# Bergvca/string_grouper

Hardware: NVIDIA H100
Metric: match_strings matched pairs/sec (663k names self-match @0.8, top 20, 3-gram) (higher is better)
Workload: dtype f64

## Files before the change

include/sg_b200.h:

```cpp
#ifndef SG_B200_H
#define SG_B200_H

#include <stddef.h>
#include <stdint.h>

#ifdef __cplusplus
extern "C" {
#endif

#define SG_OK 0
#define SG_ERR_INVALID (-1)
#define SG_ERR_CUDA (-2)
#define SG_ERR_OVERFLOW (-3)
#define SG_ERR_UNSUPPORTED (-4)

#define SG_DTYPE_F32 0
#define SG_DTYPE_F64 1

#define SG_FLAG_IGNORE_CASE 1u
#define SG_FLAG_STRIP_DEFAULT 2u

const char *sg_last_error(void);
int sg_abi_version(void);
int sg_device_info(int *sm_count, int *smem_optin_bytes, int *l2_bytes);

int64_t sg_tfidf_table_slots(int ngram);
int sg_tfidf_count(const uint8_t *bytes , const int64_t *offsets ,
                   int64_t n_docs, int ngram, unsigned flags, int32_t *df_table ,
                   uint8_t *scratch_clean , uint32_t *scratch_sort ,
                   uint32_t *scratch_key , uint32_t *scratch_tf ,
                   int32_t *row_nnz , void *stream);

size_t sg_tfidf_vocab_workspace_bytes(int64_t n_docs, int ngram);
int sg_tfidf_vocab(int64_t n_docs, int ngram, const int32_t *df_table , int32_t *rank_table ,
                   int32_t *row_nnz , int64_t *indptr ,
                   int32_t *vocab_size , int64_t *nnz_total , void *ws ,
                   size_t ws_bytes, void *stream);
int sg_tfidf_values(const int64_t *offsets , int64_t n_docs, int dtype,
                    const void *idf , const int32_t *rank_table ,
                    const uint32_t *scratch_key, const uint32_t *scratch_tf, const int32_t *row_nnz,
                    const int64_t *indptr , int32_t *indices ,
                    double *val64 , float *val32 , void *stream);

int sg_tfidf_vocab_keys(const int32_t *df_table , const int32_t *rank_table , int ngram,
                        uint32_t *keys_out , void *stream);
int sg_tfidf_vocab_df(const int32_t *df_table , const int32_t *rank_table , int ngram,
                      int32_t *df_out , void *stream);

int sg_tfidf64_count(const void *symbols , int sym_width, const int64_t *offsets ,
                     int64_t n_docs, int ngram, int bits, const uint8_t *lut ,
                     uint32_t *scratch_clean , uint64_t *scratch_sort ,
                     uint64_t *scratch_key , uint32_t *scratch_tf ,
                     int32_t *row_nnz , void *stream);
size_t sg_tfidf64_vocab_workspace_bytes(int64_t n_docs, int64_t total_symbols);
int sg_tfidf64_vocab(const int64_t *offsets , int64_t n_docs, int64_t total_symbols, int ngram, int bits,
                     const uint64_t *scratch_key, int32_t *row_nnz, int64_t *indptr ,
                     int32_t *indices , uint64_t *vocab_keys ,
                     int32_t *df , int32_t *vocab_size , int64_t *nnz_total ,
                     void *ws , size_t ws_bytes, void *stream);
int sg_tfidf64_values(const int64_t *offsets , int64_t n_docs, int dtype,
                      const void *idf , const uint32_t *scratch_tf,
                      const int64_t *indptr , const int32_t *indices ,
                      double *val64 , float *val32 , void *stream);

#define SG_SYMBOL_UNKNOWN 0xffffffffu
#define SG_LUT_UNKNOWN 0xfeu
int sg_tfidf_transform_count(const uint8_t *bytes , const int64_t *offsets ,
                             int64_t n_docs, int ngram, unsigned flags, uint8_t *scratch_clean ,
                             uint32_t *scratch_sort , uint32_t *scratch_key ,
                             uint32_t *scratch_tf , int32_t *row_nnz , void *stream);
size_t sg_tfidf_transform_workspace_bytes(int64_t n_docs);
int sg_tfidf_known(const int64_t *offsets , int64_t n_docs, const int32_t *df_table ,
                   uint32_t *scratch_key , uint32_t *scratch_tf , int32_t *row_nnz ,
                   int64_t *indptr , void *ws , size_t ws_bytes, void *stream);
int sg_tfidf64_transform_count(const void *symbols , int sym_width, const int64_t *offsets ,
                               int64_t n_docs, int ngram, int bits, const uint8_t *lut ,
                               uint32_t *scratch_clean, uint64_t *scratch_sort, uint64_t *scratch_key,
                               uint32_t *scratch_tf, int32_t *row_nnz , void *stream);
int sg_tfidf64_known(const int64_t *offsets , int64_t n_docs, const uint64_t *vocab_keys ,
                     int32_t vocab_size, const uint64_t *scratch_key , uint32_t *scratch_tf ,
// ... 325 lines not shown
```

string_grouper_b200/_device.py:

```python
import ctypes
import math
import os

import numpy as np

from . import _lib

_TORCH = None

LAUNCH_COUNTS = {"postings": 0, "candidates": 0, "rescore": 0, "select": 0, "symmetrize": 0, "tfidf": 0,
                 "rowdot": 0, "order": 0, "tiles": 0, "groups": 0, "gather": 0, "prune": 0, "dedup": 0,
                 "nearest": 0, "fields": 0}

TRANSFER_BYTES = {"d2h": 0, "h2d": 0}

DEFAULT_TILE_W = int(os.environ.get("SG_B200_TILE_W", "0"))
DEFAULT_WARPS = int(os.environ.get("SG_B200_WARPS", "8"))
GROUP_BYTES = int(os.environ.get("SG_B200_GROUP_MB", "6")) << 20
CAND_MARGIN = 1.5e-3
U16_MARGIN_PER_FEATURE = 2e-5
PRUNE_FRAC = float(os.environ.get("SG_B200_PRUNE", "0.9"))
ACC_DTYPE = os.environ.get("SG_B200_ACC", "u16")
MAX_CAND_DENSITY = float(os.environ.get("SG_B200_MAX_CAND_DENSITY", "1.5e-3"))
MAX_BUCKETS = int(os.environ.get("SG_B200_MAX_BUCKETS", str(400_000_000)))
# ... 304 lines not shown


def _build_postings(B, perm, tile_w, n_spilled=None):
    t = require_cuda()
    L = _lib.load()
    n_rows, n_cols = B.shape
    T = int(L.sg_num_tiles(n_rows, tile_w))
    nb = T * (n_cols + 1)
    if nb >= 2**31 - 1:
        raise OverflowError("posting bucket table too large: %d features x %d tiles" % (n_cols, T))
    Tp = int(L.sg_num_tiles_padded(n_rows, tile_w))
    bucket_dir = _empty(2 * nb, t.int32, B.device)
    bucket_maxw = _empty((n_cols + 1) * Tp, t.float16, B.device)
    post = _empty(max(B.nnz, 1), t.int32, B.device)
    ws_bytes = int(L.sg_postings_workspace_bytes(B.nnz, n_cols, T))
    ws = _empty(ws_bytes, t.uint8, B.device)
    w_scale = candidate_scales(1.0, B.norm_bound)[0]
    _lib.check(L.sg_postings_build(n_rows, n_cols, B.nnz, _ptr(B.d_indptr), _ptr(B.d_indices), _ptr(B.d_val32),
                                   _ptr(perm), tile_w, B.base, w_scale,
                                   _ptr(bucket_dir), _ptr(bucket_maxw), _ptr(post), _ptr(n_spilled),
                                   _ptr(ws), ws_bytes, _stream()))
    LAUNCH_COUNTS["postings"] += 5
    bound = t.zeros(Tp, dtype=t.float32, device=B.device)
    _lib.check(L.sg_tile_bounds(n_rows, _ptr(perm), _ptr(B._heavy_norm), tile_w, _ptr(bound), _stream()))
    LAUNCH_COUNTS["prune"] += 1
    return bucket_dir, bucket_maxw, post, T, bound


class DeviceMatches:

    def __init__(self, shape, row, col, score, nnz, max_row, out_dtype=np.float64, indptr=None):
        self.shape = (int(shape[0]), int(shape[1]))
        self.d_row, self.d_col, self.d_score, self.d_indptr = row, col, score, indptr
        self.nnz = int(nnz)
        self.max_row = int(max_row)
        self.out_dtype = np.dtype(out_dtype)
        self._host = None
        self.pending_fix_diagonal = False
        self.pending_mirror = False

    def with_pending(self, fix_diagonal=False, mirror=False):
        self.pending_fix_diagonal |= bool(fix_diagonal)
        self.pending_mirror |= bool(mirror)
        return self

    def host_triples(self):
        n = self.nnz
        t = torch()
        return tuple(to_host(self.d_row[:n].to(t.int64), self.d_col[:n].to(t.int64), self.d_score[:n]))

    def to_scipy(self):
        if self._host is None:
            from scipy.sparse import csr_matrix
            r, c, s = self.host_triples()
            indptr = np.zeros(self.shape[0] + 1, dtype=np.int64)
            np.cumsum(np.bincount(r, minlength=self.shape[0]), out=indptr[1:])
            idx_dtype = np.int32 if max(self.shape) < 2**31 and self.nnz < 2**31 else np.int64
            self._host = csr_matrix((s.astype(self.out_dtype, copy=False), c.astype(idx_dtype),
                                     indptr.astype(idx_dtype)), shape=self.shape)
        return self._host

    def get_shape(self):
        return self.shape

    def toarray(self):
        return self.to_scipy().toarray()

    def __getattr__(self, name):
        if name in _SCIPY_CSR_ATTRS:
            return getattr(self.to_scipy(), name)
        raise AttributeError("%s has no attribute %r" % (type(self).__name__, name))

# ... 238 lines not shown
        stats["dedup"] = groups is not None

    mark(stats, "k2_start")
    scale = A.norm_bound * B.norm_bound
    margin = CAND_MARGIN * max(scale, 1.0)
    thr_c = max(float(threshold) - margin, 0.0)
    acc = (acc or ACC_DTYPE).lower()
    if acc not in ("u16", "f32"):
        raise ValueError("accumulator dtype must be 'u16' or 'f32', got %r" % (acc,))
    if not fixed_point_ok(A, B) or thr_c < 0.05:
        acc = "f32"
    acc_code = _lib.SG_ACC_U16 if acc == "u16" else _lib.SG_ACC_F32
    margin_pf = U16_MARGIN_PER_FEATURE if acc == "u16" else 0.0
    kernel = (kernel or K2_KERNEL).lower()
    if kernel not in ("tiles", "row"):
        raise ValueError("kernel must be 'tiles' or 'row', got %r" % (kernel,))
    use_tiles = kernel == "tiles" and acc == "u16" and B.shape[1] <= int(L.sg_tiles_max_cols())
    tiles = None
    if use_tiles:
        tiles = right_tiles(B)
        if tiles["stage_bytes"] is None:
            tiles["stage_bytes"] = int(tiles["maxima"][0].item())
        smem_optin = t.cuda.get_device_properties(dev).shared_memory_per_block_optin
        tile_warps = next((w for w in (TILE_WARPS, 8) if w in (8, 16) and
                           int(L.sg_tiles_smem_bytes(tiles["stage_bytes"], w)) <= smem_optin), None)
        if tile_warps is None:
            use_tiles, tiles = False, None
    if use_tiles:
        margin = TILE_MARGIN * max(scale, 1.0)
        margin_pf = TILE_MARGIN_PER_FEATURE
    _, a_scale, b_scale = candidate_scales(A.norm_bound, B.norm_bound)
    prune_auto = prune is None
    prune = PRUNE_FRAC if prune is None else float(prune)
    counters = t.zeros(4, dtype=t.int64, device=dev)
    cap = int(os.environ.get("SG_B200_CAND_CAP", 0)) or min(96 * n_rows + (1 << 22), 1 << 30)
    if use_tiles:
        hrank, perm_b, _ = right_order(B)
        tile_w, warps, T, tile_bound = tiles["W"], tile_warps, tiles["T"], tiles["bound"]
        tiles_per_group = 0
        lpack = _empty(2 * A.d_indices.numel(), t.int32, dev)
        mask_words = int(L.sg_tiles_mask_words(n_right))
    else:
        tile_w, warps = pick_tile(n_right, tile_w, warps, 2 if acc == "u16" else 4, n_left=n_rows)
        if blocked:
            warps = 8
        while (-(-n_right // tile_w)) * (B.shape[1] + 1) > MAX_BUCKETS and tile_w < 32768:
            tile_w *= 2
        if blocked:
            hrank, perm_b, rank_b, bucket_dir, bucket_maxw, post, T, tile_bound, sorted_ids = \
                blocked_right_side(B, ids_b, tile_w)
        else:
            hrank, perm_b, _, bucket_dir, bucket_maxw, post, T, tile_bound = right_side(B, tile_w)
        tiles_per_group = max(64, int(GROUP_BYTES // max(4 * B.nnz / T, 1)) // 64 * 64)
    triangle = not nearest and A is B and row_begin == 0 and row_end == n_left
    hi_pos = None
    if blocked:
        lo_pos, hi_pos = block_ranges(sorted_ids, ids_a)
        if triangle:
            perm_a, diag_rank = perm_b, rank_b
        else:
            perm_a = blocked_order(row_order(A, hrank, row_begin, row_end, want_rank=False)[0], ids_a)
            diag_rank = lo_pos
        pair_cum = np.zeros(n_rows + 1, dtype=np.int64)
        pair_cum[1:] = to_host(t.cumsum((hi_pos - diag_rank)[perm_a.long()].long(), 0))[0]
    elif triangle:
        perm_a, diag_rank = perm_b, right_order(B)[2]
    else:
        perm_a, _ = row_order(A, hrank, row_begin, row_end, want_rank=False)
        diag_rank = None
    mark(stats, "right_side")
    c_count = ctypes.c_void_p(counters.data_ptr())
    c_queue = ctypes.c_void_p(counters.data_ptr() + 8)
    c_walk = ctypes.c_void_p(counters.data_ptr() + 16)
    c_mirror = ctypes.c_void_p(counters.data_ptr() + 24) if triangle else None
    dummy = _empty(1, t.int32, dev)
    pruned = {}
    group_items = None
    if blocked:
        group_items = _empty(2 * -(-T // tiles_per_group) + 1, t.int64, dev)
    elif triangle and not use_tiles:
        group_items = _empty(-(-T // tiles_per_group) + 1, t.int64, dev)

    def launch_tiles(perm, n, row_buf, col_buf, capacity):
        l_idx, l_val, l_len, l_thr, l_xp, _ = pruned["arrays"]
        stride = (n + 31) // 32 * 32
        rowinfo = _empty(4 * stride, t.int32, dev)
        mask = _empty(mask_words * stride, t.int32, dev)
        diag_tile_min = _empty(stride // 32, t.int32, dev) if triangle else None
        counters.zero_()
        _lib.check(L.sg_tiles_pack_left(n, _ptr(perm), 0, _ptr(A.d_indptr), _ptr(l_len), _ptr(l_idx), _ptr(l_val),
                                        _ptr(l_thr), _ptr(l_xp), max(B.norm_bound, 1.0), _ptr(lpack), _ptr(rowinfo),
                                        _stream()))
        _lib.check(L.sg_tiles_filter(n, _ptr(rowinfo), _ptr(lpack), _ptr(tiles["maxw"]), n_right, _ptr(tile_bound),
                                     _ptr(perm), _ptr(diag_rank), _ptr(diag_tile_min), _ptr(mask), stride, _stream()))
        _lib.check(L.sg_tiles_candidates(_ptr(perm), n, 0, _ptr(rowinfo), _ptr(lpack), _ptr(mask), stride,
                                         _ptr(tiles["desc"]), _ptr(tiles["blob"]), n_right, B.shape[1],
                                         _ptr(tile_bound), _ptr(perm_b), _ptr(diag_rank), _ptr(diag_tile_min),
                                         tiles["stage_bytes"], _ptr(row_buf), _ptr(col_buf), capacity, c_count,
                                         c_queue, c_walk, warps, _stream()))
        LAUNCH_COUNTS["tiles"] += 3

    def launch(perm, rb, re_, row_buf, col_buf, capacity, partial_buf=None):
        if use_tiles:
            return launch_tiles(perm, re_ - rb, row_buf, col_buf, capacity)
        l_idx, l_val, l_len, l_thr, l_xp, _ = pruned["arrays"]
        counters.zero_()
        if blocked:
            _lib.check(L.sg_cossim_candidates_range(
                _ptr(A.d_indptr), _ptr(l_len), _ptr(l_idx), _ptr(l_val), rb, re_, _ptr(perm), n_right, A.shape[1],
                _ptr(bucket_dir), _ptr(bucket_maxw), _ptr(post), _ptr(perm_b), tile_w, acc_code,
                a_scale, b_scale, thr_c, _ptr(l_thr), _ptr(l_xp), _ptr(tile_bound), tiles_per_group,
                _ptr(diag_rank), _ptr(hi_pos), _ptr(group_items), _ptr(row_buf), _ptr(col_buf), _ptr(partial_buf),
                capacity, c_count, c_queue, warps, _stream()))
            LAUNCH_COUNTS["candidates"] += 1
            return
        _lib.check(L.sg_cossim_candidates(
            _ptr(A.d_indptr), _ptr(l_len), _ptr(l_idx), _ptr(l_val), rb, re_, _ptr(perm), n_right,
            A.shape[1], _ptr(bucket_dir), _ptr(bucket_maxw), _ptr(post), _ptr(perm_b), tile_w, acc_code,
            a_scale, b_scale, thr_c, _ptr(l_thr), _ptr(l_xp), _ptr(tile_bound), tiles_per_group, _ptr(diag_rank),
            _ptr(group_items), _ptr(row_buf), _ptr(col_buf), _ptr(partial_buf), capacity, c_count, c_queue, warps,
            _stream()))
        LAUNCH_COUNTS["candidates"] += 1

    levels = [prune]
    if prune_auto and prune > 0.0 and thr_c > 0.0:
        levels = [prune, 0.75 * prune, 0.5 * prune, 0.25 * prune, 0.0]

    def prepare(level):
        if (level > 0.0 and thr_c > 0.0) or margin_pf > 0.0:
            pruned["arrays"] = prune_left(A, B, hrank, row_begin, row_end, float(threshold), margin, margin_pf,
                                          level if thr_c > 0.0 else 0.0)
        else:
            pruned["arrays"] = (A.d_indices, A.d_val32, None, None, None, None)

    def timed_launch(perm, rb, re_, row_buf, col_buf, capacity, partial_buf=None):
        if _timed(stats):
            ev0, ev1 = t.cuda.Event(enable_timing=True), t.cuda.Event(enable_timing=True)
            ev0.record()
        launch(perm, rb, re_, row_buf, col_buf, capacity, partial_buf)
        if _timed(stats):
            ev1.record()
            stats.setdefault("candidate_events", []).append((ev0, ev1))
        head = counters[:4].cpu().numpy()
        if use_tiles and stats is not None:
            stats["pairs_walked"] = stats.get("pairs_walked", 0) + int(head[2])
            stats["postings_walked"] = stats.get("postings_walked", 0) + int(head[3])
        return int(head[0])

    fixed_cap = bool(os.environ.get("SG_B200_CAND_CAP"))
    sample = None
    if not fixed_cap and n_rows >= 65536:
        stride = max(64, n_rows // 8192)
        sample = perm_a[:n_rows:stride].contiguous()
    est = None
    first = None
    search = True
    n_pairs = (float(pair_cum[-1]) if blocked else n_rows * (n_rows + 1) / 2 if triangle
               else float(n_rows) * n_right)
    dense = MAX_CAND_DENSITY * n_pairs

    def share(lo, hi):
        if blocked:
            return float(pair_cum[hi] - pair_cum[lo]) / max(n_pairs, 1.0)
        if not triangle:
            return (hi - lo) / n_rows
        return ((hi - lo) * n_rows - (lo + hi - 1) * (hi - lo) / 2) / (n_rows * (n_rows + 1) / 2)

    chunk_cand = max(CAND_CHUNK // 2, 1) if triangle else CAND_CHUNK
    refine = REFINE and not use_tiles and acc == "u16" and margin_pf > 0.0
    if not fixed_cap and (n_pairs if blocked else float(n_rows) * float(n_right)) <= OPTIMISTIC_PAIRS:
        prune = levels[0]
        prepare(prune)
        cap0 = int(min(int(dense) + (1 << 22), chunk_cand))
        cand_row0 = _empty(cap0, t.int32, dev)
        cand_col0 = _empty(cap0, t.int32, dev)
        cand_part0 = _empty(cap0, t.float32, dev) if refine else None
        mark(stats, "prune_sample")
        n0 = timed_launch(perm_a, row_begin, row_end, cand_row0, cand_col0, cap0, cand_part0)
        mark(stats, "candidates")
        too_dense = len(levels) > 1 and sample is not None and n0 > dense
        if n0 <= cap0 and not too_dense:
            first = (cand_row0, cand_col0, cand_part0, n0)
            search = False
        else:
            del cand_row0, cand_col0, cand_part0
            if _timed(stats):
                stats["wasted_launch"] = True
            if too_dense:
                levels = levels[1:]
            else:
                est, search = n0, False
    if search:
        for level in levels:
            prepare(level)
            prune = level
            if sample is None:
                break
            launch(sample, row_begin, row_begin + int(sample.numel()), dummy, dummy, 0)
            est = int(counters[0].item()) * stride
            if est <= dense:
                break
    l_idx, l_val, l_len, l_thr, l_xp, l_xg = pruned["arrays"]
    mark(stats, "prune_sample")
    if stats is not None:
        stats["prune"], stats["acc"] = prune, acc
        stats["kernel"] = "tiles" if use_tiles else "row"
        stats["n_candidates_estimate"] = est
        kept_len = (l_len[row_begin:row_end] if l_len is not None else
                    A.d_indptr[row_begin + 1:row_end + 1] - A.d_indptr[row_begin:row_end])
        stats["n_rows_long"] = int((kept_len > 32).sum().item())
        if stats.get("count_macs") and l_len is not None:
            df = feature_df(B).long()
            pos = t.arange(A.d_indices.numel(), device=dev)
            rid = t.searchsorted(A.d_indptr[:n_left + 1].contiguous(), pos, right=True) - 1
            ok = (rid >= row_begin) & (rid < row_end)
            rid = rid.clamp(0, n_left - 1)
            live = ok & ((pos - A.d_indptr[rid]) < l_len[rid].long())
            stats["macs_walked"] = int(df[l_idx.long().clamp(0, A.shape[1] - 1)][live].sum().item())
            stats["features_kept"] = int(live.sum().item())

    n_chunks = 1 if est is None else max(1, -(-int(1.3 * est) // chunk_cand))
    rows_per_chunk = -(-n_rows // n_chunks)
    kept = []
    n_cand_total = n_above = 0
    max_row_cnt = 0
    row_cnt = t.zeros(n_rows + 1, dtype=t.int32, device=dev)
    for lo in range(0, n_rows, rows_per_chunk):
        hi = min(lo + rows_per_chunk, n_rows)
        perm_chunk = perm_a if (lo == 0 and hi == n_rows) else perm_a[lo:hi]
        if est is not None:
            cap = min(max(int(1.3 * est * share(lo, hi)) + (1 << 22), 1 << 22), 1 << 31)
        for attempt in range(3):
            if first is not None:
                cand_row, cand_col, cand_part, n_cand = first
                first = None
                break
            cand_row = _empty(cap, t.int32, dev)
            cand_col = _empty(cap, t.int32, dev)
            cand_part = _empty(cap, t.float32, dev) if refine else None
            n_cand = timed_launch(perm_chunk, row_begin, row_begin + (hi - lo), cand_row, cand_col, cap, cand_part)
            if n_cand <= cap:
                break
            if n_cand * 24 > t.cuda.get_device_properties(dev).total_memory // 2:
                raise OverflowError("%d candidate pairs above the threshold do not fit the candidate buffer; "
                                    "raise min_similarity or split the input" % n_cand)
            cap = n_cand
        else:
            raise OverflowError("candidate buffer overflow")
        n_cand_total += n_cand
        mark(stats, "candidates")
        n_out = 2 * n_cand if triangle else n_cand
        score = _empty(n_out, t.float64, dev)
        keep_row = _empty(n_out, t.int32, dev)
        keep_col = _empty(n_out, t.int32, dev)
        counters.zero_()
        if nearest and refine and cand_part is not None and l_xg is not None:
            _lib.check(L.sg_rescore_refined_nearest(
                n_cand, _ptr(cand_row), _ptr(cand_col), _ptr(cand_part), _ptr(l_xg), _ptr(B._heavy_groups),
                _ptr(l_thr), _ptr(A.d_indptr), _ptr(A.d_indices), _ptr(A.d_val), _ptr(B.d_indptr), _ptr(B.d_indices),
                _ptr(B.d_val), dt, _ptr(score), float(threshold), _ptr(keep_row), _ptr(keep_col), c_count, c_walk,
                _ptr(row_best), row_begin, None, None, 0.0, 0.0, None, _stream()))
        elif nearest:
            _lib.check(L.sg_rescore_nearest(n_cand, _ptr(cand_row), _ptr(cand_col), _ptr(A.d_indptr),
                                            _ptr(A.d_indices), _ptr(A.d_val), _ptr(B.d_indptr), _ptr(B.d_indices),
                                            _ptr(B.d_val), dt, _ptr(score), float(threshold), _ptr(keep_row),
                                            _ptr(keep_col), c_count, _ptr(row_best), row_begin, None, None, _stream()))
        elif refine and cand_part is not None and l_xg is not None:
            _lib.check(L.sg_rescore_refined(n_cand, _ptr(cand_row), _ptr(cand_col), _ptr(cand_part), _ptr(l_xg),
                                            _ptr(B._heavy_groups), _ptr(l_thr), _ptr(A.d_indptr), _ptr(A.d_indices),
                                            _ptr(A.d_val), _ptr(B.d_indptr), _ptr(B.d_indices), _ptr(B.d_val), dt,
                                            _ptr(score), float(threshold), _ptr(keep_row), _ptr(keep_col), c_count,
                                            c_walk, c_mirror, _ptr(row_cnt), row_begin, _stream()))
        else:
            _lib.check(L.sg_rescore(n_cand, _ptr(cand_row), _ptr(cand_col), _ptr(A.d_indptr), _ptr(A.d_indices),
                                    _ptr(A.d_val), _ptr(B.d_indptr), _ptr(B.d_indices), _ptr(B.d_val), dt,
                                    _ptr(score), float(threshold), _ptr(keep_row), _ptr(keep_col), c_count,
                                    c_mirror, _ptr(row_cnt), row_begin, _stream()))
        LAUNCH_COUNTS["rescore"] += 1
        if lo + rows_per_chunk >= n_rows:
            _lib.check(L.sg_row_count_max(n_rows, _ptr(row_cnt), c_queue, _stream()))
        head = counters[:4].cpu().numpy()
        n_keep, max_row_cnt = int(head[0]), int(head[1])
        n_above += n_keep - int(head[3])
        if refine and stats is not None:
            stats["n_refined"] = stats.get("n_refined", 0) + int(head[2])
        mark(stats, "rescore")
        if n_chunks > 1:
            keep_row, keep_col, score = keep_row[:n_keep].clone(), keep_col[:n_keep].clone(), score[:n_keep].clone()
# ... 424 lines not shown
        LAUNCH_COUNTS["select"] += 7
        if stats is not None:
            stats["select"] = "sort"
    th = tail.cpu().numpy()
    mark(stats, "select")
    nnz = int(th[0])
    max_row = int(th[1:2].view(np.int32)[0])
    return DeviceMatches(shape, out_row, out_col, out_score, nnz, max_row, indptr=out_indptr)


def _select_groups(cand_row, cand_col, score, n_cand, groups, top_n, shape, stats):
    t = torch()
    L = _lib.load()
    dev = cand_row.device
    m, n = groups["m"], shape[0]
    grp_cnt = _empty(m, t.int32, dev)
    totals = t.zeros(2, dtype=t.int64, device=dev)
    _lib.check(L.sg_topn_groups_count(n_cand, _ptr(cand_row), _ptr(cand_col), m, _ptr(groups["mem_ptr"]), top_n,
                                      _ptr(grp_cnt), _ptr(totals), _stream()))
    n_expanded, n_out = (int(x) for x in totals.cpu().numpy())
    out_indptr = _empty(n + 1, t.int64, dev)
    out_row = _empty(n_out, t.int32, dev)
    out_col = _empty(n_out, t.int32, dev)
    out_score = _empty(n_out, t.float64, dev)
    tail = t.zeros(2, dtype=t.int64, device=dev)
    ws_bytes = int(L.sg_topn_select_groups_workspace_bytes(n_cand, n_expanded, m, n, top_n))
    ws = _empty(ws_bytes, t.uint8, dev)
    _lib.check(L.sg_topn_select_groups(n_cand, _ptr(cand_row), _ptr(cand_col), _ptr(score), m, _ptr(groups["mem_ptr"]),
                                       _ptr(groups["mem_rows"]), _ptr(grp_cnt), n_expanded, n, _ptr(groups["uid"]),
                                       top_n, _ptr(out_indptr), _ptr(out_row), _ptr(out_col), _ptr(out_score),
                                       ctypes.c_void_p(tail.data_ptr()), ctypes.c_void_p(tail.data_ptr() + 8),
                                       _ptr(ws), ws_bytes, _stream()))
    LAUNCH_COUNTS["select"] += 11 if top_n <= 32 else 13
    th = tail.cpu().numpy()
    mark(stats, "select")
    if stats is not None:
        stats["select"] = "rows"
        stats["n_unique_rows"], stats["n_expanded"] = m, n_expanded
    nnz = int(th[0])
    max_row = int(th[1:2].view(np.int32)[0])
    return DeviceMatches(shape, out_row, out_col, out_score, nnz, max_row, indptr=out_indptr)


def symmetrize(M, fix_diagonal=True, mirror=True):
    t = require_cuda()
    L = _lib.load()
    n = M.shape[0]
    dev = M.d_row.device
    flags = (_lib.SG_SYMM_FIX_DIAGONAL if fix_diagonal else 0) | (_lib.SG_SYMM_MIRROR if mirror else 0)
    cap = 2 * M.nnz + n
    out_row = _empty(cap, t.int32, dev)
    out_col = _empty(cap, t.int32, dev)
    out_score = _empty(cap, t.float64, dev)
    out_nnz = t.zeros(1, dtype=t.int64, device=dev)
    ws_bytes = int(L.sg_symmetrize_workspace_bytes(M.nnz, n))
    ws = _empty(ws_bytes, t.uint8, dev)
    _lib.check(L.sg_symmetrize(n, M.nnz, flags, _ptr(M.d_row), _ptr(M.d_col), _ptr(M.d_score), _ptr(out_row),
                               _ptr(out_col), _ptr(out_score), _ptr(out_nnz), _ptr(ws), ws_bytes, _stream()))
    LAUNCH_COUNTS["symmetrize"] += 3
    nnz = int(out_nnz.item())
    return DeviceMatches(M.shape, out_row, out_col, out_score, nnz, M.max_row, out_dtype=M.out_dtype)


def group_reps(M, n, centroid, keep_device=False):
    t = require_cuda()
    L = _lib.load()
    dev = M.d_row.device
    rep = _empty(n, t.int32, dev)
    ws_bytes = int(L.sg_group_reps_workspace_bytes(n))
    ws = _empty(ws_bytes, t.uint8, dev)
    _lib.check(L.sg_group_reps(n, M.nnz, _ptr(M.d_row), _ptr(M.d_col), _ptr(M.d_score), 1 if centroid else 0,
                               _ptr(rep), _ptr(ws), ws_bytes, _stream()))
    LAUNCH_COUNTS["groups"] += 6
    host = rep[:n].cpu().numpy().astype(np.int64)
    return (host, rep) if keep_device else host


def group_star(M, n, centroid, keep_device=False):
    t = require_cuda()
    L = _lib.load()
    dev = M.d_row.device
    rep = _empty(n, t.int32, dev)
    ws_bytes = int(L.sg_group_star_workspace_bytes(n))
    ws = _empty(ws_bytes, t.uint8, dev)
    _lib.check(L.sg_group_star(n, M.nnz, _ptr(M.d_row), _ptr(M.d_col), _ptr(M.d_score), 1 if centroid else 0,
                               _ptr(rep), _ptr(ws), ws_bytes, _stream()))
    LAUNCH_COUNTS["groups"] += 7 if centroid else 3
    host = rep[:n].cpu().numpy().astype(np.int64)
    return (host, rep) if keep_device else host


def nearest_master(M, n_right):
    t = require_cuda()
    L = _lib.load()
# ... 102 lines not shown
        k, n_rows, ptrs(*[p.d_indptr.data_ptr() for p in parts]), ptrs(*[p.d_indices.data_ptr() for p in parts]),
        ptrs(*[p.d_val.data_ptr() for p in parts]), (ctypes.c_double * k)(*[float(s) for s in scales]),
        (ctypes.c_int32 * k)(*[int(c) for c in col_off[:-1]]), _lib.SG_DTYPE_F64 if f64 else _lib.SG_DTYPE_F32,
        _ptr(indptr), _ptr(indices), _ptr(val), _ptr(val32) if f64 else None, _ptr(ws), ws_bytes, _stream()))
    LAUNCH_COUNTS["fields"] += 2
    return DeviceCSR((n_rows, int(col_off[-1])), indptr, indices, val, val32, nnz, np_dtype, 1.0)


def pair_scores(A, B, M):
    t = require_cuda()
    L = _lib.load()
    if not M.nnz:
        return np.zeros(0, np.float64)
    out = _empty(M.nnz, t.float64, M.d_row.device)
    dt = _lib.SG_DTYPE_F32 if A.dtype == np.float32 else _lib.SG_DTYPE_F64
    _lib.check(L.sg_rescore(M.nnz, _ptr(M.d_row), _ptr(M.d_col), _ptr(A.d_indptr), _ptr(A.d_indices), _ptr(A.d_val),
                            _ptr(B.d_indptr), _ptr(B.d_indices), _ptr(B.d_val), dt, _ptr(out), 0.0, None, None, None,
                            None, None, 0, _stream()))
    LAUNCH_COUNTS["rescore"] += 1
    return to_host(out[:M.nnz])[0]


def sklearn_idf(df, n_docs_fit, dtype):
    dtype = np.float32 if np.dtype(dtype) == np.float32 else np.float64
    df = np.asarray(df).astype(dtype)
    df += 1.0
    idf = np.full_like(df, fill_value=int(n_docs_fit) + 1, dtype=dtype)
    idf /= df
    np.log(idf, out=idf)
    idf += 1.0
    return idf


def _upload_idf(df_host, n_docs_fit, np_dtype, device):
    idf = sklearn_idf(df_host, n_docs_fit, np_dtype)
    TRANSFER_BYTES["h2d"] += int(idf.nbytes)
    d_idf = torch().from_numpy(idf).to(device) if len(idf) else _empty(1, torch().float64, device)
    return idf, d_idf


class DeviceVocabulary:

    alphabet = np.arange(128, dtype=np.uint32)
    bits = 7

    def __init__(self, df_table, rank_table, ngram, n_docs, vocab_size, idf=None, d_idf=None):
        self.d_df, self.d_rank = df_table, rank_table
        self.ngram, self.n_docs, self.size = int(ngram), int(n_docs), int(vocab_size)
        self.idf_, self.d_idf = idf, d_idf
        self._sorted_keys = None

    def sorted_keys(self):
        if self._sorted_keys is None:
            t = require_cuda()
            L = _lib.load()
            keys = _empty(self.size, t.int32, self.d_df.device)
            _lib.check(L.sg_tfidf_vocab_keys(_ptr(self.d_df), _ptr(self.d_rank), self.ngram, _ptr(keys), _stream()))
            self._sorted_keys = keys.to(t.int64)
            LAUNCH_COUNTS["tfidf"] += 1
        return self._sorted_keys

    def feature_names(self):
        from ._ingest import decode_vocab_keys
        t = require_cuda()
        L = _lib.load()
        keys = _empty(self.size, t.int32, self.d_df.device)
        _lib.check(L.sg_tfidf_vocab_keys(_ptr(self.d_df), _ptr(self.d_rank), self.ngram, _ptr(keys), _stream()))
        return decode_vocab_keys(keys[:self.size].cpu().numpy().view(np.uint32), self.ngram)


def upload_strings(data, offsets, device=None):
    t = require_cuda()
    device = device or t.device("cuda", t.cuda.current_device())
    total = int(offsets[-1])
    d_bytes = (t.from_numpy(np.ascontiguousarray(data)).to(device, non_blocking=True) if total
               else _empty(1, t.uint8, device))
    d_off = t.from_numpy(np.ascontiguousarray(offsets, dtype=np.int64)).to(device, non_blocking=True)
    return d_bytes, d_off, total


class DeviceVocabulary64:

    def __init__(self, keys, df, alphabet, bits, ngram, n_docs, vocab_size, idf=None, d_idf=None):
# ... 111 lines not shown
    slots = int(L.sg_tfidf_table_slots(int(ngram)))
    if slots < 0:
        raise NotImplementedError("ngram_size=%r: the device vectoriser supports 1 <= ngram_size <= 4" % (ngram,))
    np_dtype = np.float32 if np.dtype(dtype) == np.float32 else np.float64
    df = t.zeros(slots, dtype=t.int32, device=device)
    rank = _empty(slots, t.int32, device)
    s_clean = _empty(total, t.uint8, device)
    s_sort = _empty(total, t.int32, device)
    s_key = _empty(total, t.int32, device)
    s_tf = _empty(total, t.int32, device)
    row_nnz = _empty(n_docs + 1, t.int32, device)
    _lib.check(L.sg_tfidf_count(_ptr(d_bytes), _ptr(d_off), n_docs, int(ngram), int(flags), _ptr(df), _ptr(s_clean),
                                _ptr(s_sort), _ptr(s_key), _ptr(s_tf), _ptr(row_nnz), _stream()))
    if df_allreduce is not None:
        df_allreduce(df)
    indptr = _empty(n_docs + 1, t.int64, device)
    indices = _empty(total, t.int32, device)
    val32 = _empty(total, t.float32, device)
    val64 = _empty(total, t.float64, device) if np_dtype == np.float64 else None
    tail = t.zeros(2, dtype=t.int64, device=device)
    ws_bytes = int(L.sg_tfidf_vocab_workspace_bytes(n_docs, int(ngram)))
    ws = _empty(ws_bytes, t.uint8, device)
    dt = _lib.SG_DTYPE_F32 if np_dtype == np.float32 else _lib.SG_DTYPE_F64
    _lib.check(L.sg_tfidf_vocab(n_docs, int(ngram), _ptr(df), _ptr(rank), _ptr(row_nnz), _ptr(indptr),
                                ctypes.c_void_p(tail.data_ptr()), ctypes.c_void_p(tail.data_ptr() + 8), _ptr(ws),
                                ws_bytes, _stream()))
    n_master = int(n_master)
    head = t.cat([tail, indptr[n_master:n_master + 1]]).cpu().numpy()
    V = int(head[0:1].view(np.int32)[0])
    nnz = int(head[1])
    split = int(head[2])
    n_fit = n_docs if n_docs_fit is None else int(n_docs_fit)
    col_df = _empty(max(V, 1), t.int32, device)
    _lib.check(L.sg_tfidf_vocab_df(_ptr(df), _ptr(rank), int(ngram), _ptr(col_df), _stream()))
    idf, d_idf = _upload_idf(to_host(col_df[:V])[0], n_fit, np_dtype, device)
    _lib.check(L.sg_tfidf_values(_ptr(d_off), n_docs, dt, _ptr(d_idf), _ptr(rank), _ptr(s_key), _ptr(s_tf),
                                 _ptr(row_nnz), _ptr(indptr), _ptr(indices), _ptr(val64), _ptr(val32), _stream()))
    LAUNCH_COUNTS["tfidf"] += 5
    val = val64 if np_dtype == np.float64 else val32
    vocab = DeviceVocabulary(df, rank, ngram, n_fit, V, idf, d_idf)
    if stats is not None:
        stats.update(n_docs=n_docs, total_bytes=total, nnz=nnz, vocab=V)
    master = DeviceCSR((n_master, V), indptr[:n_master + 1], indices, val, val32, split, np_dtype, 1.0, base=0)
    master.nnz_parent = nnz
    if n_master == n_docs:
        if df_allreduce is None and n_docs_fit is None:
            master._df = col_df
        return master, None, vocab
    dup = DeviceCSR((n_docs - n_master, V), indptr[n_master:], indices, val, val32, nnz - split, np_dtype, 1.0,
                    base=split)
    dup.nnz_parent = nnz
    return master, dup, vocab


def tfidf_transform(data, offsets, n_first, flags, vocab, stats=None):
    t = require_cuda()
    L = _lib.load()
    from . import _ingest
    device = vocab.d_idf.device
    n_docs = len(offsets) - 1
    total = int(offsets[-1])
    np_dtype = np.dtype(vocab.idf_.dtype)
    dt = _lib.SG_DTYPE_F32 if np_dtype == np.float32 else _lib.SG_DTYPE_F64
    V = vocab.size
    row_nnz = _empty(n_docs + 1, t.int32, device)
    indptr = _empty(n_docs + 1, t.int64, device)
    indices = _empty(total, t.int32, device)
    val32 = _empty(total, t.float32, device)
    val64 = _empty(total, t.float64, device) if np_dtype == np.float64 else None
    ws_bytes = int(L.sg_tfidf_transform_workspace_bytes(n_docs))
    ws = _empty(ws_bytes, t.uint8, device)
    if isinstance(vocab, DeviceVocabulary) and data.dtype == np.uint8:
        d_bytes, d_off, _ = upload_strings(data, offsets, device)
        h2d = int(total + 8 * len(offsets))
        s_clean = _empty(total, t.uint8, device)
        s_sort = _empty(total, t.int32, device)
        s_key = _empty(total, t.int32, device)
        s_tf = _empty(total, t.int32, device)
        _lib.check(L.sg_tfidf_transform_count(_ptr(d_bytes), _ptr(d_off), n_docs, vocab.ngram, int(flags),
                                              _ptr(s_clean), _ptr(s_sort), _ptr(s_key), _ptr(s_tf), _ptr(row_nnz),
                                              _stream()))
        _lib.check(L.sg_tfidf_known(_ptr(d_off), n_docs, _ptr(vocab.d_df), _ptr(s_key), _ptr(s_tf), _ptr(row_nnz),
                                    _ptr(indptr), _ptr(ws), ws_bytes, _stream()))
        _lib.check(L.sg_tfidf_values(_ptr(d_off), n_docs, dt, _ptr(vocab.d_idf), _ptr(vocab.d_rank), _ptr(s_key),
                                     _ptr(s_tf), _ptr(row_nnz), _ptr(indptr), _ptr(indices), _ptr(val64), _ptr(val32),
                                     _stream()))
        LAUNCH_COUNTS["tfidf"] += 3
        form = "dense key table"
    else:
        keys = vocab.sorted_keys()
        if data.dtype == np.uint8:
            sym_width = 1
            d_sym = t.from_numpy(np.ascontiguousarray(data)).to(device) if total else _empty(1, t.uint8, device)
            d_lut = t.from_numpy(_ingest.fitted_byte_lut(data, flags, vocab.alphabet)).to(device)
        else:
# ... 85 lines not shown
```

string_grouper_b200/_lib.py:

```python
import ctypes
import os

_HERE = os.path.dirname(os.path.abspath(__file__))
SO_PATH = os.path.join(_HERE, "libsg_b200.so")

SG_OK = 0
SG_ERR_INVALID = -1
SG_ERR_CUDA = -2
SG_ERR_OVERFLOW = -3
SG_ERR_UNSUPPORTED = -4
SG_DTYPE_F32 = 0
SG_DTYPE_F64 = 1
SG_FLAG_IGNORE_CASE = 1
SG_FLAG_STRIP_DEFAULT = 2
SG_SYMM_FIX_DIAGONAL = 1
SG_SYMM_MIRROR = 2
SG_ACC_F32 = 0
SG_ACC_U16 = 1
SG_FLOOR_SEED = 1
SG_FLOOR_LONG_ROWS = 2
SG_SYMBOL_UNKNOWN = 0xffffffff
SG_LUT_UNKNOWN = 0xfe
SG_FIELDS_MAX = 32

_i64 = ctypes.c_int64
_i32 = ctypes.c_int
_p = ctypes.c_void_p
_sz = ctypes.c_size_t
_f32 = ctypes.c_float
_f64 = ctypes.c_double
_u32 = ctypes.c_uint

SIGNATURES = {
    "sg_last_error": (ctypes.c_char_p, []),
    "sg_abi_version": (_i32, []),
    "sg_device_info": (_i32, [_p, _p, _p]),
    "sg_tfidf_table_slots": (_i64, [_i32]),
    "sg_tfidf_count": (_i32, [_p, _p, _i64, _i32, _u32, _p, _p, _p, _p, _p, _p, _p]),
    "sg_tfidf_vocab_workspace_bytes": (_sz, [_i64, _i32]),
    "sg_tfidf_vocab": (_i32, [_i64, _i32, _p, _p, _p, _p, _p, _p, _p, _sz, _p]),
    "sg_tfidf_values": (_i32, [_p, _i64, _i32, _p, _p, _p, _p, _p, _p, _p, _p, _p, _p]),
    "sg_tfidf_vocab_keys": (_i32, [_p, _p, _i32, _p, _p]),
    "sg_tfidf_vocab_df": (_i32, [_p, _p, _i32, _p, _p]),
    "sg_tfidf64_count": (_i32, [_p, _i32, _p, _i64, _i32, _i32, _p, _p, _p, _p, _p, _p, _p]),
    "sg_tfidf64_vocab_workspace_bytes": (_sz, [_i64, _i64]),
    "sg_tfidf64_vocab": (_i32, [_p, _i64, _i64, _i32, _i32, _p, _p, _p, _p, _p, _p, _p, _p, _p, _sz, _p]),
    "sg_tfidf64_values": (_i32, [_p, _i64, _i32, _p, _p, _p, _p, _p, _p, _p]),
    "sg_tfidf_transform_count": (_i32, [_p, _p, _i64, _i32, _u32, _p, _p, _p, _p, _p, _p]),
    "sg_tfidf_transform_workspace_bytes": (_sz, [_i64]),
    "sg_tfidf_known": (_i32, [_p, _i64, _p, _p, _p, _p, _p, _p, _sz, _p]),
    "sg_tfidf64_transform_count": (_i32, [_p, _i32, _p, _i64, _i32, _i32, _p, _p, _p, _p, _p, _p, _p]),
    "sg_tfidf64_known": (_i32, [_p, _i64, _p, _i32, _p, _p, _p, _p, _p, _p, _p, _sz, _p]),
    "sg_num_tiles": (_i64, [_i64, _i32]),
    "sg_num_tiles_padded": (_i64, [_i64, _i32]),
    "sg_postings_workspace_bytes": (_sz, [_i64, _i64, _i64]),
    "sg_postings_build": (_i32, [_i64, _i64, _i64, _p, _p, _p, _p, _i32, _i64, _f32, _p, _p, _p, _p, _p, _sz, _p]),
    "sg_feature_df": (_i32, [_i64, _i64, _p, _p, _p, _p]),
    "sg_prune_rows": (_i32, [_i64, _i64, _p, _p, _p, _p, _p, _f32, _f32, _f32, _f32, _f32, _p, _p, _p, _p, _p, _p, _p]),
    "sg_prune_rows_floor": (_i32, [_i64, _i64, _p, _p, _p, _p, _p, _f32, _f32, _f32, _p, _f32, _f32, _p, _p, _p, _p,
                                   _p, _p, _p]),
    "sg_heavy_norms": (_i32, [_i64, _i64, _p, _p, _p, _p, _p, _p, _p]),
    "sg_tile_bounds": (_i32, [_i64, _p, _p, _i32, _p, _p]),
    "sg_cossim_candidates": (_i32, [_p, _p, _p, _p, _i64, _i64, _p, _i64, _i64, _p, _p, _p, _p, _i32, _i32, _f32,
                                    _f32, _f32, _p, _p, _p, _i64, _p, _p, _p, _p, _p, _i64, _p, _p, _i32, _p]),
    "sg_cossim_candidates_floor": (_i32, [_p, _p, _p, _p, _i64, _i64, _p, _i64, _i64, _p, _p, _p, _p, _i32, _i32,
                                          _f32, _f32, _f32, _p, _p, _p, _i64, _p, _p, _p, _i64, _p, _p, _i32, _p, _i32,
                                          _f32, _f32, _p, _i32, _p]),
    "sg_cossim_candidates_range": (_i32, [_p, _p, _p, _p, _i64, _i64, _p, _i64, _i64, _p, _p, _p, _p, _i32, _i32,
                                          _f32, _f32, _f32, _p, _p, _p, _i64, _p, _p, _p, _p, _p, _p, _i64, _p, _p, _i32,
                                          _p]),
    "sg_cossim_candidates_range_floor": (_i32, [_p, _p, _p, _p, _i64, _i64, _p, _i64, _i64, _p, _p, _p, _p, _i32,
                                                _i32, _f32, _f32, _f32, _p, _p, _p, _i64, _p, _p, _p, _p, _p, _p, _i64,
                                                _p, _p, _i32, _p, _i32, _f32, _f32, _p, _i32, _p]),
    "sg_tiles_tile_w": (_i32, []),
    "sg_tiles_max_cols": (_i64, []),
    "sg_tiles_blob_bound": (_i64, [_i64, _i64, _i64]),
# ... 91 lines not shown
```

string_grouper_b200/csrc/sg_tfidf.cu:

```cuda
#include <cub/cub.cuh>

#include "sg_common.cuh"

namespace sg {

constexpr int K1_WARPS = 8;
constexpr int K1_CAP = 256;

__device__ __forceinline__ bool is_stripped(unsigned c) {
    return (c >= 0x2cu && c <= 0x2fu) || (c >= 0x09u && c <= 0x0du) || (c >= 0x1cu && c <= 0x20u);
}

__device__ void warp_sort_keys(uint32_t *keys, int G, int lane) {
    if (G < 2) return;
    int P = 2;
    while (P < G) P <<= 1;
    const int half = P >> 1;
    for (int k = 2; k <= P; k <<= 1) {
        const int hk = k >> 1;
        for (int i = lane; i < half; i += 32) {
            const int blk = i / hk, o = i - blk * hk;
            const int a = blk * k + o, b = blk * k + (k - 1 - o);
            if (b < G) {
                const uint32_t ka = keys[a], kb = keys[b];
// ... 155 lines not shown
    for (int64_t doc = (int64_t)blockIdx.x * K1_WARPS + warp; doc < n_docs; doc += (int64_t)gridDim.x * K1_WARPS) {
        const int nnz = row_nnz[doc];
        if (nnz == 0) continue;
        const int64_t s = offsets[doc], o = indptr[doc];
        double sum = 0.0;
        for (int base = 0; base < nnz; base += 32) {
            const int i = base + lane;
            double sq = 0.0;
            if (i < nnz) {
                const T x = (T)scratch_tf[s + i] * idf[rank[scratch_key[s + i]]];
                sq = NormMath<T>::sq(x);
            }
            const int m = nnz - base < 32 ? nnz - base : 32;
            for (int l = 0; l < m; ++l) sum = __dadd_rn(sum, __shfl_sync(FULL, sq, l));
        }
        const double norm = __dsqrt_rn(sum);
        for (int i = lane; i < nnz; i += 32) {
            const int32_t c = rank[scratch_key[s + i]];
            T x = (T)scratch_tf[s + i] * idf[c];
            if (sum != 0.0) x = NormMath<T>::scale(x, norm);
            indices[o + i] = c;
            if (val64) val64[o + i] = (double)x;
            val32[o + i] = (float)x;
        }
    }
}

__global__ void vocab_keys_kernel(int64_t slots, const int32_t *__restrict__ df, const int32_t *__restrict__ rank,
                                  uint32_t *__restrict__ keys_out) {
    const int64_t i = (int64_t)blockIdx.x * blockDim.x + threadIdx.x;
    if (i < slots && df[i] > 0) keys_out[rank[i]] = (uint32_t)i;
}

__global__ void vocab_df_kernel(int64_t slots, const int32_t *__restrict__ df, const int32_t *__restrict__ rank,
                                int32_t *__restrict__ df_out) {
    const int64_t i = (int64_t)blockIdx.x * blockDim.x + threadIdx.x;
    if (i < slots && df[i] > 0) df_out[rank[i]] = df[i];
}

static int k1_grid(int64_t n_docs, unsigned *grid_out) {
    int dev = 0, n_sm = 0;
    SG_CUDA_TRY(cudaGetDevice(&dev));
    SG_CUDA_TRY(cudaDeviceGetAttribute(&n_sm, cudaDevAttrMultiProcessorCount, dev));
    int64_t grid = (n_docs + K1_WARPS - 1) / K1_WARPS;
    const int64_t cap = (int64_t)n_sm * 8;
    *grid_out = (unsigned)(grid > cap ? cap : grid);
    return SG_OK;
}

template <bool kDf>
static int launch_count(const uint8_t *bytes, const int64_t *offsets, int64_t n_docs, int ngram, unsigned flags,
                        int32_t *df_table, uint8_t *scratch_clean, uint32_t *scratch_sort, uint32_t *scratch_key,
                        uint32_t *scratch_tf, int32_t *row_nnz, cudaStream_t st) {
    if (ngram < 1 || ngram > 4)
        return fail(SG_ERR_UNSUPPORTED, "ngram_size %d: the device vectoriser packs 7-bit characters into 32-bit keys "
                                        "and supports 1 <= ngram_size <= 4", ngram);
    if (n_docs <= 0) return SG_OK;
    unsigned grid = 0;
    const int rc = k1_grid(n_docs, &grid);
    if (rc != SG_OK) return rc;
    tfidf_count_kernel<kDf><<<grid, K1_WARPS * 32, 0, st>>>(bytes, offsets, n_docs, ngram, flags, df_table,
                                                            scratch_clean, scratch_sort, scratch_key, scratch_tf,
                                                            row_nnz);
    SG_LAUNCH_CHECK();
    return SG_OK;
}

int transform_indptr(int64_t n_docs, int32_t *row_nnz, int64_t *indptr, void *ws, size_t ws_bytes, cudaStream_t st) {
    size_t b = 0;
    cub::DeviceScan::ExclusiveScan(nullptr, b, (int32_t *)nullptr, (int64_t *)nullptr, cub::Sum(), (int64_t)0,
// ... 92 lines not shown
                    const int64_t *indptr, int32_t *indices, double *val64, float *val32, void *stream_) {
    cudaStream_t st = (cudaStream_t)stream_;
    if (dtype != SG_DTYPE_F32 && dtype != SG_DTYPE_F64) return fail(SG_ERR_INVALID, "bad dtype");
    if (dtype == SG_DTYPE_F64 && !val64) return fail(SG_ERR_INVALID, "val64 is required for float64");
    if (n_docs <= 0) return SG_OK;
    int dev = 0, n_sm = 0;
    SG_CUDA_TRY(cudaGetDevice(&dev));
    SG_CUDA_TRY(cudaDeviceGetAttribute(&n_sm, cudaDevAttrMultiProcessorCount, dev));
    int64_t grid = (n_docs + K1_WARPS - 1) / K1_WARPS;
    const int64_t cap = (int64_t)n_sm * 8;
    if (grid > cap) grid = cap;
    if (dtype == SG_DTYPE_F64)
        tfidf_values_kernel<double><<<(unsigned)grid, K1_WARPS * 32, 0, st>>>(
            offsets, n_docs, (const double *)idf, rank_table, scratch_key, scratch_tf, row_nnz, indptr, indices, val64,
            val32);
    else
        tfidf_values_kernel<float><<<(unsigned)grid, K1_WARPS * 32, 0, st>>>(
            offsets, n_docs, (const float *)idf, rank_table, scratch_key, scratch_tf, row_nnz, indptr, indices,
            nullptr, val32);
    SG_LAUNCH_CHECK();
    return SG_OK;
}

int sg_tfidf_vocab_keys(const int32_t *df_table, const int32_t *rank_table, int ngram, uint32_t *keys_out,
                        void *stream_) {
    cudaStream_t st = (cudaStream_t)stream_;
    const int64_t slots = sg_tfidf_table_slots(ngram);
    if (slots < 0) return fail(SG_ERR_UNSUPPORTED, "ngram_size %d unsupported (1..4)", ngram);
    vocab_keys_kernel<<<(unsigned)((slots + 255) / 256), 256, 0, st>>>(slots, df_table, rank_table, keys_out);
    SG_LAUNCH_CHECK();
    return SG_OK;
}

int sg_tfidf_vocab_df(const int32_t *df_table, const int32_t *rank_table, int ngram, int32_t *df_out, void *stream_) {
    cudaStream_t st = (cudaStream_t)stream_;
    const int64_t slots = sg_tfidf_table_slots(ngram);
    if (slots < 0) return fail(SG_ERR_UNSUPPORTED, "ngram_size %d unsupported (1..4)", ngram);
    vocab_df_kernel<<<(unsigned)((slots + 255) / 256), 256, 0, st>>>(slots, df_table, rank_table, df_out);
    SG_LAUNCH_CHECK();
    return SG_OK;
}

}
```

Measured before the change: 256.6 million.

## Compute IDF on device from a cached per-df table and defer host syncs

Replaces the device-to-host df copy, host IDF computation and re-upload with a kernel that looks up IDF from a cached table indexed by document frequency. It also makes DeviceMatches nnz/max_row lazy device scalars so select_rows and symmetrize no longer force a sync, and folds the long-row count into the counters readback. This removes several blocking round trips in the pipeline, at the cost of a small cached table per (n_fit, dtype, device) and lazy host materialization of idf_.

```diff
diff --git a/include/sg_b200.h b/include/sg_b200.h
--- a/include/sg_b200.h
+++ b/include/sg_b200.h
@@ -44,8 +44,9 @@
 
 int sg_tfidf_vocab_keys(const int32_t *df_table , const int32_t *rank_table , int ngram,
                         uint32_t *keys_out , void *stream);
-int sg_tfidf_vocab_df(const int32_t *df_table , const int32_t *rank_table , int ngram,
-                      int32_t *df_out , void *stream);
+int sg_tfidf_vocab_idf(const int32_t *df_table , const int32_t *rank_table , int ngram, int dtype,
+                       const void *idf_of_df , int64_t n_fit,
+                       int32_t *df_out , void *idf_out , void *stream);
 
 int sg_tfidf64_count(const void *symbols , int sym_width, const int64_t *offsets ,
                      int64_t n_docs, int ngram, int bits, const uint8_t *lut ,
diff --git a/string_grouper_b200/_device.py b/string_grouper_b200/_device.py
--- a/string_grouper_b200/_device.py
+++ b/string_grouper_b200/_device.py
@@ -360,12 +360,24 @@
     def __init__(self, shape, row, col, score, nnz, max_row, out_dtype=np.float64, indptr=None):
         self.shape = (int(shape[0]), int(shape[1]))
         self.d_row, self.d_col, self.d_score, self.d_indptr = row, col, score, indptr
-        self.nnz = int(nnz)
-        self.max_row = int(max_row)
+        self._nnz = nnz if hasattr(nnz, "device") else int(nnz)
+        self._max_row = max_row if hasattr(max_row, "device") else int(max_row)
         self.out_dtype = np.dtype(out_dtype)
         self._host = None
         self.pending_fix_diagonal = False
         self.pending_mirror = False
+
+    @property
+    def nnz(self):
+        if not isinstance(self._nnz, int):
+            self._nnz = int(self._nnz.item())
+        return self._nnz
+
+    @property
+    def max_row(self):
+        if not isinstance(self._max_row, int):
+            self._max_row = int(self._max_row.item())
+        return self._max_row
 
     def with_pending(self, fix_diagonal=False, mirror=False):
         self.pending_fix_diagonal |= bool(fix_diagonal)
@@ -670,7 +682,7 @@
     _, a_scale, b_scale = candidate_scales(A.norm_bound, B.norm_bound)
     prune_auto = prune is None
     prune = PRUNE_FRAC if prune is None else float(prune)
-    counters = t.zeros(4, dtype=t.int64, device=dev)
+    counters = t.zeros(5, dtype=t.int64, device=dev)
     cap = int(os.environ.get("SG_B200_CAND_CAP", 0)) or min(96 * n_rows + (1 << 22), 1 << 30)
     if use_tiles:
         hrank, perm_b, _ = right_order(B)
@@ -725,7 +737,7 @@
         rowinfo = _empty(4 * stride, t.int32, dev)
         mask = _empty(mask_words * stride, t.int32, dev)
         diag_tile_min = _empty(stride // 32, t.int32, dev) if triangle else None
-        counters.zero_()
+        counters[:4].zero_()
         _lib.check(L.sg_tiles_pack_left(n, _ptr(perm), 0, _ptr(A.d_indptr), _ptr(l_len), _ptr(l_idx), _ptr(l_val),
                                         _ptr(l_thr), _ptr(l_xp), max(B.norm_bound, 1.0), _ptr(lpack), _ptr(rowinfo),
                                         _stream()))
@@ -742,7 +754,7 @@
         if use_tiles:
             return launch_tiles(perm, re_ - rb, row_buf, col_buf, capacity)
         l_idx, l_val, l_len, l_thr, l_xp, _ = pruned["arrays"]
-        counters.zero_()
+        counters[:4].zero_()
         if blocked:
             _lib.check(L.sg_cossim_candidates_range(
                 _ptr(A.d_indptr), _ptr(l_len), _ptr(l_idx), _ptr(l_val), rb, re_, _ptr(perm), n_right, A.shape[1],
@@ -770,6 +782,11 @@
                                           level if thr_c > 0.0 else 0.0)
         else:
             pruned["arrays"] = (A.d_indices, A.d_val32, None, None, None, None)
+        if stats is not None:
+            l_len = pruned["arrays"][2]
+            kept_len = (l_len[row_begin:row_end] if l_len is not None else
+                        A.d_indptr[row_begin + 1:row_end + 1] - A.d_indptr[row_begin:row_end])
+            counters[4] = (kept_len > 32).sum()
 
     def timed_launch(perm, rb, re_, row_buf, col_buf, capacity, partial_buf=None):
         if _timed(stats):
@@ -779,10 +796,12 @@
         if _timed(stats):
             ev1.record()
             stats.setdefault("candidate_events", []).append((ev0, ev1))
-        head = counters[:4].cpu().numpy()
-        if use_tiles and stats is not None:
-            stats["pairs_walked"] = stats.get("pairs_walked", 0) + int(head[2])
-            stats["postings_walked"] = stats.get("postings_walked", 0) + int(head[3])
+        head = counters.cpu().numpy()
+        if stats is not None:
+            stats["n_rows_long"] = int(head[4])
+            if use_tiles:
+                stats["pairs_walked"] = stats.get("pairs_walked", 0) + int(head[2])
+                stats["postings_walked"] = stats.get("postings_walked", 0) + int(head[3])
         return int(head[0])
 
     fixed_cap = bool(os.environ.get("SG_B200_CAND_CAP"))
@@ -844,9 +863,6 @@
         stats["prune"], stats["acc"] = prune, acc
         stats["kernel"] = "tiles" if use_tiles else "row"
         stats["n_candidates_estimate"] = est
-        kept_len = (l_len[row_begin:row_end] if l_len is not None else
-                    A.d_indptr[row_begin + 1:row_end + 1] - A.d_indptr[row_begin:row_end])
-        stats["n_rows_long"] = int((kept_len > 32).sum().item())
         if stats.get("count_macs") and l_len is not None:
             df = feature_df(B).long()
             pos = t.arange(A.d_indices.numel(), device=dev)
@@ -891,7 +907,7 @@
         score = _empty(n_out, t.float64, dev)
         keep_row = _empty(n_out, t.int32, dev)
         keep_col = _empty(n_out, t.int32, dev)
-        counters.zero_()
+        counters[:4].zero_()
         if nearest and refine and cand_part is not None and l_xg is not None:
             _lib.check(L.sg_rescore_refined_nearest(
                 n_cand, _ptr(cand_row), _ptr(cand_col), _ptr(cand_part), _ptr(l_xg), _ptr(B._heavy_groups),
@@ -1382,14 +1398,12 @@
                                        ctypes.c_void_p(tail.data_ptr()), ctypes.c_void_p(tail.data_ptr() + 8),
                                        _ptr(ws), ws_bytes, _stream()))
     LAUNCH_COUNTS["select"] += 11 if top_n <= 32 else 13
-    th = tail.cpu().numpy()
     mark(stats, "select")
     if stats is not None:
         stats["select"] = "rows"
         stats["n_unique_rows"], stats["n_expanded"] = m, n_expanded
-    nnz = int(th[0])
-    max_row = int(th[1:2].view(np.int32)[0])
-    return DeviceMatches(shape, out_row, out_col, out_score, nnz, max_row, indptr=out_indptr)
+    return DeviceMatches(shape, out_row, out_col, out_score, n_out, tail[1:2].view(t.int32)[:1],
+                         indptr=out_indptr)
 
 
 def symmetrize(M, fix_diagonal=True, mirror=True):
@@ -1408,8 +1422,7 @@
     _lib.check(L.sg_symmetrize(n, M.nnz, flags, _ptr(M.d_row), _ptr(M.d_col), _ptr(M.d_score), _ptr(out_row),
                                _ptr(out_col), _ptr(out_score), _ptr(out_nnz), _ptr(ws), ws_bytes, _stream()))
     LAUNCH_COUNTS["symmetrize"] += 3
-    nnz = int(out_nnz.item())
-    return DeviceMatches(M.shape, out_row, out_col, out_score, nnz, M.max_row, out_dtype=M.out_dtype)
+    return DeviceMatches(M.shape, out_row, out_col, out_score, out_nnz, M._max_row, out_dtype=M.out_dtype)
 
 
 def group_reps(M, n, centroid, keep_device=False):
@@ -1578,6 +1591,21 @@
     return idf
 
 
+_IDF_TABLES = {}
+
+
+def idf_table(n_fit, np_dtype, device):
+    key = (int(n_fit), np.dtype(np_dtype).str, str(device))
+    d = _IDF_TABLES.get(key)
+    if d is None:
+        if len(_IDF_TABLES) >= 4:
+            _IDF_TABLES.clear()
+        tab = sklearn_idf(np.arange(int(n_fit) + 1), n_fit, np_dtype)
+        TRANSFER_BYTES["h2d"] += int(tab.nbytes)
+        d = _IDF_TABLES[key] = torch().from_numpy(tab).to(device)
+    return d
+
+
 def _upload_idf(df_host, n_docs_fit, np_dtype, device):
     idf = sklearn_idf(df_host, n_docs_fit, np_dtype)
     TRANSFER_BYTES["h2d"] += int(idf.nbytes)
@@ -1593,8 +1621,14 @@
     def __init__(self, df_table, rank_table, ngram, n_docs, vocab_size, idf=None, d_idf=None):
         self.d_df, self.d_rank = df_table, rank_table
         self.ngram, self.n_docs, self.size = int(ngram), int(n_docs), int(vocab_size)
-        self.idf_, self.d_idf = idf, d_idf
+        self._idf, self.d_idf = idf, d_idf
         self._sorted_keys = None
+
+    @property
+    def idf_(self):
+        if self._idf is None:
+            self._idf = to_host(self.d_idf[:self.size])[0]
+        return self._idf
 
     def sorted_keys(self):
         if self._sorted_keys is None:
@@ -1772,13 +1806,14 @@
     split = int(head[2])
     n_fit = n_docs if n_docs_fit is None else int(n_docs_fit)
     col_df = _empty(max(V, 1), t.int32, device)
-    _lib.check(L.sg_tfidf_vocab_df(_ptr(df), _ptr(rank), int(ngram), _ptr(col_df), _stream()))
-    idf, d_idf = _upload_idf(to_host(col_df[:V])[0], n_fit, np_dtype, device)
+    d_idf = _empty(max(V, 1), t.float64 if np_dtype == np.float64 else t.float32, device)
+    _lib.check(L.sg_tfidf_vocab_idf(_ptr(df), _ptr(rank), int(ngram), dt, _ptr(idf_table(n_fit, np_dtype, device)),
+                                    n_fit, _ptr(col_df), _ptr(d_idf), _stream()))
     _lib.check(L.sg_tfidf_values(_ptr(d_off), n_docs, dt, _ptr(d_idf), _ptr(rank), _ptr(s_key), _ptr(s_tf),
                                  _ptr(row_nnz), _ptr(indptr), _ptr(indices), _ptr(val64), _ptr(val32), _stream()))
     LAUNCH_COUNTS["tfidf"] += 5
     val = val64 if np_dtype == np.float64 else val32
-    vocab = DeviceVocabulary(df, rank, ngram, n_fit, V, idf, d_idf)
+    vocab = DeviceVocabulary(df, rank, ngram, n_fit, V, None, d_idf)
     if stats is not None:
         stats.update(n_docs=n_docs, total_bytes=total, nnz=nnz, vocab=V)
     master = DeviceCSR((n_master, V), indptr[:n_master + 1], indices, val, val32, split, np_dtype, 1.0, base=0)
@@ -1800,7 +1835,7 @@
     device = vocab.d_idf.device
     n_docs = len(offsets) - 1
     total = int(offsets[-1])
-    np_dtype = np.dtype(vocab.idf_.dtype)
+    np_dtype = np.dtype(np.float32 if vocab.d_idf.dtype == torch().float32 else np.float64)
     dt = _lib.SG_DTYPE_F32 if np_dtype == np.float32 else _lib.SG_DTYPE_F64
     V = vocab.size
     row_nnz = _empty(n_docs + 1, t.int32, device)
diff --git a/string_grouper_b200/_lib.py b/string_grouper_b200/_lib.py
--- a/string_grouper_b200/_lib.py
+++ b/string_grouper_b200/_lib.py
@@ -41,7 +41,7 @@
     "sg_tfidf_vocab": (_i32, [_i64, _i32, _p, _p, _p, _p, _p, _p, _p, _sz, _p]),
     "sg_tfidf_values": (_i32, [_p, _i64, _i32, _p, _p, _p, _p, _p, _p, _p, _p, _p, _p]),
     "sg_tfidf_vocab_keys": (_i32, [_p, _p, _i32, _p, _p]),
-    "sg_tfidf_vocab_df": (_i32, [_p, _p, _i32, _p, _p]),
+    "sg_tfidf_vocab_idf": (_i32, [_p, _p, _i32, _i32, _p, _i64, _p, _p, _p]),
     "sg_tfidf64_count": (_i32, [_p, _i32, _p, _i64, _i32, _i32, _p, _p, _p, _p, _p, _p, _p]),
     "sg_tfidf64_vocab_workspace_bytes": (_sz, [_i64, _i64]),
     "sg_tfidf64_vocab": (_i32, [_p, _i64, _i64, _i32, _i32, _p, _p, _p, _p, _p, _p, _p, _p, _p, _sz, _p]),
diff --git a/string_grouper_b200/csrc/sg_tfidf.cu b/string_grouper_b200/csrc/sg_tfidf.cu
--- a/string_grouper_b200/csrc/sg_tfidf.cu
+++ b/string_grouper_b200/csrc/sg_tfidf.cu
@@ -211,10 +211,16 @@
     if (i < slots && df[i] > 0) keys_out[rank[i]] = (uint32_t)i;
 }
 
-__global__ void vocab_df_kernel(int64_t slots, const int32_t *__restrict__ df, const int32_t *__restrict__ rank,
-                                int32_t *__restrict__ df_out) {
+template <typename T>
+__global__ void vocab_idf_kernel(int64_t slots, const int32_t *__restrict__ df, const int32_t *__restrict__ rank,
+                                 const T *__restrict__ idf_of_df, int64_t n_fit, int32_t *__restrict__ df_out,
+                                 T *__restrict__ idf_out) {
     const int64_t i = (int64_t)blockIdx.x * blockDim.x + threadIdx.x;
-    if (i < slots && df[i] > 0) df_out[rank[i]] = df[i];
+    if (i >= slots) return;
+    const int32_t d = df[i];
+    if (d <= 0) return;
+    df_out[rank[i]] = d;
+    idf_out[rank[i]] = d <= n_fit ? idf_of_df[d] : (T)NAN;
 }
 
 static int k1_grid(int64_t n_docs, unsigned *grid_out) {
@@ -373,13 +379,22 @@
     return SG_OK;
 }
 
-int sg_tfidf_vocab_df(const int32_t *df_table, const int32_t *rank_table, int ngram, int32_t *df_out, void *stream_) {
+int sg_tfidf_vocab_idf(const int32_t *df_table, const int32_t *rank_table, int ngram, int dtype, const void *idf_of_df,
+                       int64_t n_fit, int32_t *df_out, void *idf_out, void *stream_) {
     cudaStream_t st = (cudaStream_t)stream_;
     const int64_t slots = sg_tfidf_table_slots(ngram);
     if (slots < 0) return fail(SG_ERR_UNSUPPORTED, "ngram_size %d unsupported (1..4)", ngram);
-    vocab_df_kernel<<<(unsigned)((slots + 255) / 256), 256, 0, st>>>(slots, df_table, rank_table, df_out);
-    SG_LAUNCH_CHECK();
-    return SG_OK;
-}
-
-}
+    if (dtype != SG_DTYPE_F32 && dtype != SG_DTYPE_F64) return fail(SG_ERR_INVALID, "bad dtype");
+    if (n_fit < 0) return fail(SG_ERR_INVALID, "need n_fit >= 0");
+    const unsigned grid = (unsigned)((slots + 255) / 256);
+    if (dtype == SG_DTYPE_F64)
+        vocab_idf_kernel<double><<<grid, 256, 0, st>>>(slots, df_table, rank_table, (const double *)idf_of_df, n_fit,
+                                                       df_out, (double *)idf_out);
+    else
+        vocab_idf_kernel<float><<<grid, 256, 0, st>>>(slots, df_table, rank_table, (const float *)idf_of_df, n_fit,
+                                                      df_out, (float *)idf_out);
+    SG_LAUNCH_CHECK();
+    return SG_OK;
+}
+
+}
```

After: 272.3 million, median of 6. 6.1% higher.
